# azrael417/mlperf-deepcam

Hardware: AMD Instinct MI355X
Metric: samples/sec (768x1152x16) train step (higher is better)
Workload: dtype bf16; 1 GPU; DeepLabV3+/Xception train step (fwd + weighted CE + bwd + LAMB), 768x1152x16, local_batch=8, bf16 activations / fp32 master weights, random-init seed 333; local_batch=8, global_batch=8, parallelism=dp1, optimizer=LAMB, hip_graph=False, launch_list_replay=False

## Files before the change

mlperf-deepcam_amd/csrc/igemm224.hip:

```cpp
#include <type_traits>

#include "igemm.h"

namespace dc {

namespace {

constexpr int NWS = 3, NPS = 3;
constexpr int NPB = 7;
constexpr int PW224_AUXP = 0;

typedef __attribute__((address_space(1))) const void* gas_ptr;
typedef __attribute__((address_space(3))) void* lds_ptr;
typedef __attribute__((ext_vector_type(2))) uint32_t u32x2;
typedef __attribute__((ext_vector_type(4))) uint32_t u32x4;

__device__ inline uint32_t swap_rows16(uint32_t v) { return (uint32_t)__builtin_amdgcn_ds_swizzle((int)v, 0x401F); }
__device__ inline float row_sum16(float v) {
  v += __int_as_float(__builtin_amdgcn_update_dpp(0, __float_as_int(v), 0xB1, 0xF, 0xF, true));
  v += __int_as_float(__builtin_amdgcn_update_dpp(0, __float_as_int(v), 0x4E, 0xF, 0xF, true));
  v += __int_as_float(__builtin_amdgcn_update_dpp(0, __float_as_int(v), 0x141, 0xF, 0xF, true));
  v += __int_as_float(__builtin_amdgcn_update_dpp(0, __float_as_int(v), 0x140, 0xF, 0xF, true));
  return v;
}

__device__ inline void mfma_v(f32x4& c, const bf16x8& av, const bf16x8& bv) {
  asm volatile("v_mfma_f32_16x16x32_bf16 %0, %1, %2, %0" : "+v"(c) : "v"(av), "v"(bv));
}
template <int OFF>
__device__ inline void lds_read16(bf16x8& dst, uint32_t addr) {
  static_assert(OFF >= 0 && OFF < 65536, "ds_read offset field");
  asm volatile("ds_read_b128 %0, %1 offset:%2" : "=v"(dst) : "v"(addr), "n"(OFF) : "memory");
}
template <int OFF>
__device__ inline void lds_read_tr(u32x4& dst, uint32_t addr) {
  static_assert(OFF >= 0 && OFF + 512 < 65536, "ds_read offset field");
  u32x2 lo, hi;
  asm volatile("ds_read_b64_tr_b16 %0, %1 offset:%2" : "=v"(lo) : "v"(addr), "n"(OFF) : "memory");
  asm volatile("ds_read_b64_tr_b16 %0, %1 offset:%2" : "=v"(hi) : "v"(addr), "n"(OFF + 512) : "memory");
  dst[0] = lo[0]; dst[1] = lo[1]; dst[2] = hi[0]; dst[3] = hi[1];
}
template <int N>
__device__ inline void lgkm_wait() {
  asm volatile("s_waitcnt lgkmcnt(%0)" ::"n"(N) : "memory");
}
template <int N>
__device__ inline void vm_lgkm0_wait() {
  asm volatile("s_waitcnt vmcnt(%0) lgkmcnt(0)" ::"n"(N) : "memory");
}

template <int I, int N, typename F>
__device__ inline void static_for(F&& f) {
  if constexpr (I < N) {
    f(std::integral_constant<int, I>{});
    static_for<I + 1, N>(f);
  }
}

template <int TN_>
struct Cfg {
  static constexpr int TN = TN_;
  static constexpr int GP = 2;
  static constexpr int GC = 8 / GP;
  static constexpr int NCB = TN / 16 / GC;
  static constexpr int TM = GP * NPB * 16;
  static constexpr int WSTG = 32 * TN * 2;
  static constexpr int NWI = WSTG / 1024;
  static constexpr int WSLOTS = (NWI + 7) / 8;
  static constexpr int WDEF = (NWI % 8) ? 1 : 0;
  static constexpr int PSTG = TM * 128;
  static constexpr int NPI = PSTG / 1024;
  static constexpr int PSLOTS = (NPI + 7) / 8;
  static constexpr int HP = PSLOTS / 2;
  static constexpr int POFF = NWS * WSTG;
  static constexpr int RING = NWS * WSTG + NPS * PSTG;
  static_assert(PSLOTS % 2 == 0 && NCB % 3 == 0 && RING <= 160 * 1024, "plan");
  static_assert(NPI - 8 * (PSLOTS - 1) == 4 && (WDEF == 0 || NWI - 8 * (WSLOTS - 1) == 4), "waves 0..3 own every last slot");
};

template <int TNT>
__global__ __launch_bounds__(512) void pw224_kernel(const IgemmParams p) {
  typedef Cfg<TNT> K;
  constexpr int NCB = K::NCB, GC = K::GC, HP = K::HP, TN = K::TN, WSTG = K::WSTG, GP = K::GP;
  extern __shared__ __attribute__((aligned(16))) char smem[];
  const GatherGeom& g = p.g;
  const int tid = threadIdx.x, lane = tid & 63;
  const int wave = __builtin_amdgcn_readfirstlane(tid >> 6);
  const int grp = wave / GC;
  const int wc = wave % GC;
  const bool late = wave >= 4;

  const int ntn = (g.Cout + TN - 1) / TN;
  const int nwg = gridDim.x;
  const int q8 = nwg >> 3, r8 = nwg & 7, xcd = blockIdx.x & 7, xslot = blockIdx.x >> 3;
  const int tile = (xcd < r8 ? xcd * (q8 + 1) : r8 * (q8 + 1) + (xcd - r8) * q8) + xslot;
  const int tm = tile / ntn;
  const int n0 = (tile % ntn) * TN, m0 = tm * K::TM;
  const int nsteps = (g.Cin + 31) / 32;

  const int krow = 8 * (wave & 3) + (lane >> 3);
  const int wkey = ((krow >> 1) & 1) | (((krow >> 3) & 1) << 1);
  unsigned srcw[K::WSLOTS], srcp[K::PSLOTS];
#pragma unroll
  for (int i = 0; i < K::WSLOTS; ++i) {
    const int ncol = ((wave >> 2) + 2 * i) * 64 + ((((lane & 7) >> 1) ^ wkey) << 4) + (lane & 1) * 8;
    srcw[i] = (unsigned)(((size_t)krow * p.ldw_kn + n0 + ncol) * 2);
// ... 77 lines not shown
        static_for<0, ND>([&](auto kc) {
          constexpr int k = decltype(kc)::value;
          if constexpr (EB[k] == i) { if (!late) dma_k(kc); }
          if constexpr (LB[k] == i) { if (late) dma_k(kc); }
        });
      }
      if constexpr (i == NCB - 1) {
        if (dma) {
          if (has_last) vm_lgkm0_wait<K::WSLOTS + HP>(); else vm_lgkm0_wait<K::WSLOTS + HP - K::WDEF - H>();
        } else {
          vm_lgkm0_wait<0>();
        }
        __builtin_amdgcn_s_barrier();
        lds_read_tr<0>(fa[0], wnxt + a_base[0] - lds0);
        lds_read_tr<0>(fa[1], wnxt + a_base[1] - lds0);
      }
      static_for<0, NPB>([&](auto jc) {
        constexpr int j = decltype(jc)::value;
        if constexpr (i == 0) lgkm_wait<NPB - 1 - j + 2>();
        else if constexpr (j == 0 && i < NCB - 2) lgkm_wait<4>();
        else if constexpr (j == 0 && i == NCB - 2) lgkm_wait<2>();
        mfma_v(acc[i][j], __builtin_bit_cast(bf16x8, fa[i % 3]), fb[j]);
        if constexpr (i == NCB - 1) lds_read16<j * 2048>(fb[j], bnxt);
      });
    });
  };

  constexpr int LATE_PRIO = 1;
  if (late) __builtin_amdgcn_s_setprio(LATE_PRIO);
#pragma unroll
  for (int q = 0; q < 2; ++q) {
#pragma unroll
    for (int i = 0; i < K::PSLOTS; ++i)
      if (i < K::PSLOTS - 1 || has_last) issue_p(i, q, K::POFF + q * K::PSTG);
#pragma unroll
    for (int i = 0; i < K::WSLOTS; ++i)
      if (i < K::WSLOTS - K::WDEF || has_last) issue_w(i, q, q * WSTG);
  }
  if (has_last) asm volatile("s_waitcnt vmcnt(%0)" ::"n"(K::WSLOTS + K::PSLOTS) : "memory");
  else asm volatile("s_waitcnt vmcnt(%0)" ::"n"(K::WSLOTS - K::WDEF + K::PSLOTS - 1) : "memory");
  __builtin_amdgcn_s_barrier();
  lds_read_tr<0>(fa[0], a_base[0]);
  lds_read_tr<0>(fa[1], a_base[1]);
  static_for<0, NPB>([&](auto jc) { lds_read16<decltype(jc)::value * 2048>(fb[decltype(jc)::value], lds0 + b_off); });
  {
    int s = 0;
    uint32_t w0 = 0, w1 = WSTG, w2 = 2 * WSTG;
    uint32_t p0 = 0, p1 = K::PSTG, p2 = 2 * K::PSTG;
    typedef std::integral_constant<int, 0> H0;
    typedef std::integral_constant<int, 1> H1;
    while (true) {
      step(H0{}, lds0 + w0, lds0 + w1, lds0 + ((b_off + p0) ^ 64), s, s + 2 < nsteps, w2, K::POFF + p2);
      if (++s == nsteps) break;
      step(H1{}, lds0 + w1, lds0 + w2, lds0 + b_off + p1, s, s + 2 < nsteps, w0, K::POFF + p2);
      if (++s == nsteps) break;
      { const uint32_t t = w0; w0 = w2; w2 = w1; w1 = t; }
      { const uint32_t t = p0; p0 = p1; p1 = p2; p2 = t; }
    }
  }
  asm volatile("s_waitcnt vmcnt(0) lgkmcnt(0)" ::: "memory");

  __builtin_amdgcn_s_barrier();

  const bool odd = fg & 1;
  bf16* __restrict__ yg = reinterpret_cast<bf16*>(p.y);
  const bool do_stats = p.slab != nullptr;
  float* red = reinterpret_cast<float*>(smem);
#pragma unroll
  for (int pr = 0; pr < NCB / 2; ++pr) {
    const int i0 = 2 * pr;
    const int cpair = TN == 384 ? ((wc >> 1) + 2 * pr) * 64 + (wc & 1) * 32 : 48 * wc;
    const int chl = cpair + (odd ? 16 : 0) + (fg >> 1) * 8;
    const int ch0 = n0 + chl;
    const bool chok = ch0 < g.Cout;
    float ba[4] = {0.f, 0.f, 0.f, 0.f}, bb[4] = {0.f, 0.f, 0.f, 0.f};
    if (p.bias != nullptr) {
#pragma unroll
      for (int r = 0; r < 4; ++r) {
        const int ca = n0 + cpair + fg * 4 + r, cb = ca + 16;
        if (ca < g.Cout) ba[r] = p.bias[ca];
        if (cb < g.Cout) bb[r] = p.bias[cb];
      }
    }
    float st[2][8];
#pragma unroll
    for (int e = 0; e < 8; ++e) st[0][e] = st[1][e] = 0.f;
#pragma unroll
    for (int j = 0; j < NPB; ++j) {
      const int m = m0 + grp * (NPB * 16) + j * 16 + fr;
      const uint32_t a0 = pack2_bf16(acc[i0][j][0] + ba[0], acc[i0][j][1] + ba[1]);
      const uint32_t a1 = pack2_bf16(acc[i0][j][2] + ba[2], acc[i0][j][3] + ba[3]);
      const uint32_t b0 = pack2_bf16(acc[i0 + 1][j][0] + bb[0], acc[i0 + 1][j][1] + bb[1]);
      const uint32_t b1 = pack2_bf16(acc[i0 + 1][j][2] + bb[2], acc[i0 + 1][j][3] + bb[3]);
      const uint32_t r0 = swap_rows16(odd ? a0 : b0), r1 = swap_rows16(odd ? a1 : b1);
      vec16 v;
      v.w[0] = odd ? r0 : a0;
      v.w[1] = odd ? r1 : a1;
      v.w[2] = odd ? b0 : r0;
      v.w[3] = odd ? b1 : r1;
      if (m < p.M && chok) {
        bf16* dst = yg + (size_t)m * p.ldy + ch0;
        float f[8];
        unpack(v, f, bf16());
        if (p.accumulate) {
          float o[8];
          unpack(ldg16(dst), o, bf16());
#pragma unroll
          for (int e = 0; e < 8; ++e) f[e] += o[e];
          pack(v, f, bf16());
          unpack(v, f, bf16());
        }
        stg16(dst, v);
        if (do_stats) {
#pragma unroll
          for (int e = 0; e < 8; ++e) {
            st[0][e] += f[e];
            st[1][e] = fmaf(f[e], f[e], st[1][e]);
          }
        }
      }
    }
    if (do_stats) {
      float mine = 0.f;
#pragma unroll
      for (int w = 0; w < 2; ++w)
#pragma unroll
        for (int e = 0; e < 8; ++e) {
          const float t = row_sum16(st[w][e]);
          if (fr == w * 8 + e) mine = t;
        }
      red[(grp * 2 + (fr >> 3)) * TN + chl + (fr & 7)] = mine;
    }
  }
  if constexpr (NCB & 1) {
    constexpr int i2 = NCB - 1;
    const int chl = 48 * wc + 32 + (fg >> 1) * 8;
    const int ch0 = n0 + chl;
    const bool chok = ch0 < g.Cout;
    float ba[4] = {0.f, 0.f, 0.f, 0.f};
    if (p.bias != nullptr) {
#pragma unroll
      for (int r = 0; r < 4; ++r) {
        const int ca = n0 + 48 * wc + 32 + fg * 4 + r;
        if (ca < g.Cout) ba[r] = p.bias[ca];
      }
    }
    float st[2][8];
#pragma unroll
    for (int e = 0; e < 8; ++e) st[0][e] = st[1][e] = 0.f;
#pragma unroll
    for (int jj = 0; jj < (NPB + 1) / 2; ++jj) {
      const int j0 = 2 * jj, j1 = 2 * jj + 1 < NPB ? 2 * jj + 1 : 2 * jj;
      const bool has1 = 2 * jj + 1 < NPB;
      const uint32_t a0 = pack2_bf16(acc[i2][j0][0] + ba[0], acc[i2][j0][1] + ba[1]);
      const uint32_t a1 = pack2_bf16(acc[i2][j0][2] + ba[2], acc[i2][j0][3] + ba[3]);
      const uint32_t b0 = pack2_bf16(acc[i2][j1][0] + ba[0], acc[i2][j1][1] + ba[1]);
      const uint32_t b1 = pack2_bf16(acc[i2][j1][2] + ba[2], acc[i2][j1][3] + ba[3]);
      const uint32_t r0 = swap_rows16(odd ? a0 : b0), r1 = swap_rows16(odd ? a1 : b1);
      vec16 v;
      v.w[0] = odd ? r0 : a0;
      v.w[1] = odd ? r1 : a1;
      v.w[2] = odd ? b0 : r0;
      v.w[3] = odd ? b1 : r1;
      const int m = m0 + grp * (NPB * 16) + (odd ? j1 : j0) * 16 + fr;
      if (m < p.M && chok && (!odd || has1)) {
        bf16* dst = yg + (size_t)m * p.ldy + ch0;
        float f[8];
        unpack(v, f, bf16());
        if (p.accumulate) {
          float o[8];
          unpack(ldg16(dst), o, bf16());
#pragma unroll
          for (int e = 0; e < 8; ++e) f[e] += o[e];
          pack(v, f, bf16());
          unpack(v, f, bf16());
        }
        stg16(dst, v);
        if (do_stats) {
#pragma unroll
          for (int e = 0; e < 8; ++e) {
            st[0][e] += f[e];
            st[1][e] = fmaf(f[e], f[e], st[1][e]);
          }
        }
      }
    }
    if (do_stats) {
      float mine = 0.f;
#pragma unroll
      for (int w = 0; w < 2; ++w)
#pragma unroll
        for (int e = 0; e < 8; ++e) {
          const float both = st[w][e] + __uint_as_float(swap_rows16(__float_as_uint(st[w][e])));
          const float t = row_sum16(both);
          if (fr == w * 8 + e) mine = t;
        }
      if (!odd) red[(grp * 2 + (fr >> 3)) * TN + chl + (fr & 7)] = mine;
    }
  }
  if (do_stats) {
    __syncthreads();
    const int rows = p.mtiles, ntm = (p.M + K::TM - 1) / K::TM;
    for (int i = tid; i < 2 * TN; i += 512) {
      const int c = i % TN, which = i / TN;
      if (n0 + c < g.Cout) {
        float v = red[which * TN + c];
#pragma unroll
        for (int gq = 1; gq < GP; ++gq) v += red[(gq * 2 + which) * TN + c];
        if (rows < 0) {
          unsafeAtomicAdd(reinterpret_cast<double*>(p.slab) + (size_t)which * g.Cout + n0 + c, (double)v);
          continue;
        }
        float* col = p.slab + (size_t)which * rows * g.Cout + n0 + c;
        col[(size_t)tm * g.Cout] = v;
        for (int r = tm + ntm; r < rows; r += ntm) col[(size_t)r * g.Cout] = 0.f;
      }
    }
  }
}

}

bool pw224_eligible(const IgemmParams& p) {
  const GatherGeom& g = p.g;
  return p.w_kn != nullptr && g.ntaps == 1 && g.os == 1 && g.is == 1 && g.taps[0].dy == 0 && g.taps[0].dx == 0 && p.m_beg == 0 && p.ngroup <= 1 &&
         g.Cin >= 128 && g.Cin % 8 == 0 && g.Cout % 8 == 0 && (((uintptr_t)p.w_kn) & 15) == 0 &&
         ((size_t)p.M + 224) * p.ldx * 2 < (1ull << 31) && ((size_t)g.Cin + 64) * p.ldw_kn * 2 < (1ull << 31);
}

int launch_pw224(const IgemmParams& p, int tn, hipStream_t st) {
  auto k384 = &pw224_kernel<384>;
  auto k192 = &pw224_kernel<192>;
  DC_ONCE({
    (void)hipFuncSetAttribute(reinterpret_cast<const void*>(k384), hipFuncAttributeMaxDynamicSharedMemorySize, Cfg<384>::RING);
    (void)hipFuncSetAttribute(reinterpret_cast<const void*>(k192), hipFuncAttributeMaxDynamicSharedMemorySize, Cfg<192>::RING);
  });
  if (tn == 192) hipLaunchKernelGGL(k192, dim3((unsigned)pw224_tiles(p, 192)), dim3(512), Cfg<192>::RING, st, p);
  else hipLaunchKernelGGL(k384, dim3((unsigned)pw224_tiles(p, 384)), dim3(512), Cfg<384>::RING, st, p);
  DC_CHECK_LAUNCH();
  return 0;
}

}
```

mlperf-deepcam_amd/engine.py:

```python
from __future__ import annotations

import ctypes as C
import math
from typing import Callable, Dict, List, Optional

import torch

from . import lib as L
from . import spec as S

BN_EPS = 1e-5
BN_MOMENTUM = 0.1
S_STEM_W = "xception_features.conv1.weight"
ACT_ALIGN = 64
BN_FIN_MAX_M = 16384
WGRAD_GROUP = 12


class Act:

    def __init__(self, eng: "Engine", name: str, N: int, H: int, W: int, Cc: int, parent: "Act" = None, off: int = 0,
                 dtype=None):
        self.eng, self.name, self.N, self.H, self.W, self.C = eng, name, N, H, W, Cc
        self.parent, self.off = parent, off
# ... 48 lines not shown
            init = init or a.grad_init
            a = a.parent
        self.grad_init = True
        self.grad_takes += 1
        return 1 if init else 0


class LazyAct:

    def __init__(self, y: Act, scale: torch.Tensor, shift: torch.Tensor, mean: torch.Tensor, invstd: torch.Tensor, relu: bool,
                 fin: Optional[dict], name: str):
        self.y, self.scale, self.shift, self.mean, self.invstd, self.relu, self.name = y, scale, shift, mean, invstd, relu, name
        self.N, self.H, self.W, self.C = y.N, y.H, y.W, y.C
        self._grad: Optional[Act] = None
        self.grad_init = False
        self.fin = fin
        self.fused_bwd: Optional[tuple] = None
        self.apply_by: Optional[Callable] = None

    @property
    def M(self) -> int:
        return self.y.M

    @property
    def grad(self) -> Act:
        if self._grad is None:
            self._grad = Act(self.y.eng, "d" + self.name, self.N, self.H, self.W, self.C, dtype=self.y.buf.dtype)
        return self._grad

    def take_grad_mode(self) -> int:
        mode = 1 if self.grad_init else 0
        self.grad_init = True
        return mode


class Engine:
    def __init__(self, batch: int, height: int, width: int, dtype=torch.bfloat16, device=None, n_input: int = 16,
                 n_classes: int = 3, seed: Optional[int] = 333, share_from: "Engine" = None, layout: "S.Layout" = None,
                 builder: Callable[["Engine"], None] = None, frozen_bn: bool = False, fuse_bn_into_head: bool = True):
        if not torch.cuda.is_available():
            raise L.DeepcamHipError("mlperf_deepcam_amd.Engine needs a HIP device: there is no CPU path")
        L.load()
        assert n_classes == 3, "the fused loss / head kernels are built for the 3 DeepCAM classes"
        assert height % 16 == 0 and width % 16 == 0, "input extents must be multiples of the output stride (16)"
        self.B, self.H, self.W = batch, height, width
        self.dtype, self.dt = dtype, L.dtype_code(dtype)
        self.device = device or torch.device("cuda", torch.cuda.current_device())
        self.n_input, self.n_classes = n_input, n_classes
        self.layout = layout if layout is not None else S.Layout(n_input, n_classes)
        self._builder = builder
        lay = self.layout
        self.act_bytes = 0
        self.saved: Dict[str, torch.Tensor] = {}
        self.saved_channels: Dict[str, int] = {}

        if share_from is not None:
            assert share_from.layout.n_params == lay.n_params and share_from.device == self.device
            self.params, self.grads, self.buffers, self.nbt = share_from.params, share_from.grads, share_from.buffers, share_from.nbt
            self.version = share_from.version
            self.grads_live = share_from.grads_live
        else:
            host = torch.empty(lay.n_params, dtype=torch.float32)
            if layout is None:
                S.init_arena(lay, host, seed)
            else:
                host.zero_()
            self.params = host.to(self.device)
            self.grads = torch.zeros(lay.n_params, dtype=torch.float32, device=self.device)
            hb = torch.zeros(lay.n_buffers, dtype=torch.float32)
            for name, (off, c) in lay.buffers.items():
                if name.endswith("running_var"):
                    hb[off:off + c] = 1.0
            self.buffers = hb.to(self.device)
            self.nbt = torch.zeros(len(lay.nbt), dtype=torch.int64, device=self.device)
            self.version = [0]
            self.grads_live = [False]
        self.packed_version = -1
        self._keep: List[torch.Tensor] = []
        self.frozen_bn = frozen_bn
        self.fuse_bn = not frozen_bn
        self.fuse_bn_into_head = fuse_bn_into_head and self.fuse_bn and dtype == torch.bfloat16
        self._sum_arena = None
        self._sum_used = 0
        self._wg_recs: List[dict] = []
        self._fold_seq: List[tuple] = []
        self._final_fold = None
        self._deferred_names: List[str] = []
        self._ready_now: List[str] = []
        self._stem_out: Optional[Act] = None
        self._layout_op: Optional[Callable[[], None]] = None
        self._layout_forked = False

        self.fwd_train: List[Callable[[], None]] = []
        self.fwd_eval: List[Callable[[], None]] = []
        self.bwd: List[Callable[[], None]] = []
        self.pack_ops: List[Callable[[], None]] = []
        self._pack_entries: List[L.PackEntry] = []
        self.grad_ready: List[List[str]] = []
        self.ws_bytes = 0
        self._ws_users: List[Callable[[], int]] = []
        self.x_in: Optional[torch.Tensor] = None
        self.x0: Optional[Act] = None
        self.x_static = torch.empty((batch, n_input, height, width), dtype=torch.float32, device=self.device)
        self.logits = torch.empty((batch, n_classes, height, width), dtype=torch.float32, device=self.device)
        self.dlogits = torch.empty_like(self.logits)
        self._build()
        self.workspace = torch.empty(max(self.ws_bytes, 256), dtype=torch.uint8, device=self.device)
        arr = (L.PackEntry * len(self._pack_entries))(*self._pack_entries)
        raw = torch.frombuffer(bytearray(bytes(arr)), dtype=torch.uint8).clone()
        self._pack_table = raw.to(self.device)
        npk = len(self._pack_entries)
        self.pack_ops.append(lambda: L.call("dc_pack_all", self.dt, L.dptr(self._pack_table), npk, self._st()))
        self.side = torch.cuda.Stream(device=self.device)
        self.workspace2 = torch.empty(max(self.ws_bytes, 256), dtype=torch.uint8, device=self.device)
        self.use_side_stream = True
        self.on_grad_ready: Optional[Callable[[List[str]], None]] = None
        self.region_marks: Optional[list] = None
        self.loss_args: Optional[dict] = None

    def pptr(self, name: str) -> C.c_void_p:
        return C.c_void_p(self.params.data_ptr() + self.layout.params[name].offset * 4)

    def gptr(self, name: str) -> C.c_void_p:
        return C.c_void_p(self.grads.data_ptr() + self.layout.params[name].offset * 4)

    def bptr(self, name: str) -> C.c_void_p:
        return C.c_void_p(self.buffers.data_ptr() + self.layout.buffers[name][0] * 4)

    def param_view(self, name: str) -> torch.Tensor:
        p = self.layout.params[name]
        return self.params[p.offset:p.offset + math.prod(p.shape)].view(p.shape)

    def grad_view(self, name: str) -> torch.Tensor:
        p = self.layout.params[name]
        return self.grads[p.offset:p.offset + math.prod(p.shape)].view(p.shape)

    def buffer_view(self, name: str) -> torch.Tensor:
        if name in self.layout.nbt:
            return self.nbt[self.layout.nbt[name]]
        off, c = self.layout.buffers[name]
        return self.buffers[off:off + c]

    def _need_ws(self, nbytes: int) -> None:
        self.ws_bytes = max(self.ws_bytes, int(nbytes))

    def _wsptr(self) -> C.c_void_p:
        return C.c_void_p(self.workspace.data_ptr())

    def _on_side(self, fn: Callable[[C.c_void_p], None]) -> None:
        if not self.use_side_stream:
            fn(self._wsptr())
            return
        L.call("dc_stream_fence", L.stream_ptr(), C.c_void_p(self.side.cuda_stream))
        with torch.cuda.stream(self.side):
            fn(C.c_void_p(self.workspace2.data_ptr()))

    @staticmethod
    def _st():
        return L.stream_ptr()

    def _f32(self, n: int) -> torch.Tensor:
        return torch.empty(n, dtype=torch.float32, device=self.device)

    SUM_ARENA_FLOATS = 1 << 21

    def _sum_row(self, channels: int) -> torch.Tensor:
        if self._sum_arena is None:
            self._sum_arena = torch.zeros(self.SUM_ARENA_FLOATS, dtype=torch.float32, device=self.device)
        n = (4 * channels + 15) // 16 * 16
        if self._sum_used + n > self.SUM_ARENA_FLOATS:
            raise L.DeepcamHipError("the arena of BatchNorm sum rows is full (Engine.SUM_ARENA_FLOATS)")
        row = self._sum_arena[self._sum_used:self._sum_used + n]
        self._sum_used += n
        return row

    def _conv(self, x: Act, wname: str, cout: int, k: int = 1, stride: int = 1, pad: int = 0, dil: int = 1,
              transposed: bool = False, out: Act = None, stats: bool = True, bias: str = None, name: str = None,
              need_dx: bool = True, f32: bool = False, fwd_group: list = None, sole_consumer: bool = False, bn_fuse: bool = False,
              sum_row: bool = True):
        lib = L.load()
        dt, tdtype = (L.DC_F32, torch.float32) if f32 else (self.dt, self.dtype)
        d = L.ConvDesc(dt, 3 if transposed else k, stride, pad, dil, 1 if transposed else 0, x.C, cout)
        ho, wo = C.c_int(), C.c_int()
        L.call("dc_conv_out_hw", C.byref(d), x.H, x.W, C.byref(ho), C.byref(wo))
        y = out or Act(self, name or wname, x.N, ho.value, wo.value, cout, dtype=tdtype)
        assert (y.H, y.W, y.C) == (ho.value, wo.value, cout) and y.buf.dtype == tdtype and x.buf.dtype == tdtype
        nwf, nwb = C.c_size_t(), C.c_size_t()
        L.call("dc_conv_packed_elems", C.byref(d), C.byref(nwf), C.byref(nwb))
        wf = torch.empty(nwf.value, dtype=tdtype, device=self.device)
        wb = torch.empty(nwb.value, dtype=tdtype, device=self.device) if need_dx else None
        both = k == 1 and stride == 1 and not transposed and not f32 and need_dx and dt == L.DC_BF16
        rows = (lib.dc_conv_stat_rows_kn if both else lib.dc_conv_stat_rows)(C.byref(d), x.N, x.H, x.W) if stats else 0
        slab = self._f32(2 * rows * cout) if stats else None
        if (stats and both and sum_row and self.fuse_bn and fwd_group is None and bias is None and out is None
                and lib.dc_conv_sum_row_kn(C.byref(d), x.N, x.H, x.W) == 1):
            rows, slab = -1, self._sum_row(cout)
        if (bn_fuse and self.fuse_bn and k == 1 and stride == 1 and not transposed and bias is None and not f32 and need_dx
                and out is None and x.parent is None):
            frows = lib.dc_pw_bn_bwd_rows(dt, x.C, cout, x.M)
            if frows > 0:
                y.pw_fuse = {"rows": frows, "taken": False}
        N, H, W = x.N, x.H, x.W
        pw, gw = self.pptr(wname), self.gptr(wname)
        pb = self.pptr(bias) if bias else None
        if f32 and self.dt != L.DC_F32:
            self.pack_ops.append(lambda: L.call("dc_conv_pack_weights", C.byref(d), pw, L.dptr(wf), L.dptr(wb), self._st()))
        else:
            self._pack_entries.append(L.PackEntry(pw.value, wf.data_ptr(), wb.data_ptr() if wb is not None else None, x.C, cout,
                                                  d.k * d.k, 1 if transposed else 0))
            self._keep += [wf] + ([wb] if wb is not None else [])

        assert both == (k == 1 and stride == 1 and not transposed and not f32 and wb is not None and dt == L.DC_BF16)

        def fwd(train: bool):
            if both:
                L.call("dc_conv_fwd_kn", C.byref(d), N, H, W, x.ptr, x.ld, L.dptr(wf), L.dptr(wb), pb, y.ptr, y.ld,
                       L.dptr(slab) if train else None, rows, 0, self._st())
            else:
                L.call("dc_conv_fwd", C.byref(d), N, H, W, x.ptr, x.ld, L.dptr(wf), pb, y.ptr, y.ld,
                       L.dptr(slab) if train else None, 0, self._st())

        if fwd_group is not None:
            assert k == 3 and stride == 1 and pad == dil and not transposed and bias is None and not f32
            fwd_group.append((dil, wf, y, slab, d, x))
        else:
            self.fwd_train.append(lambda: fwd(True))
            self.fwd_eval.append(lambda: fwd(False))
            y.conv_fwd = {"wf": wf, "slab": slab, "rows": rows, "plain": k == 1 and stride == 1 and not transposed and bias is None and not f32 and out is None}

        def make_bwd():
            pwf = y.pw_fuse
            if pwf is not None and pwf["taken"]:
                mode = x.take_grad_mode()
                assert mode == 0, f"{wname}: the fused backward pass writes the input gradient first"
                dx, do = x.grad, pwf["do"]
                frows = pwf["rows"]
                fslab = self._f32(frows * cout * x.C)
                ready = [wname] + pwf["names"]
                self._fold_seq.append(("dw", L.FoldEntry(fslab.data_ptr(), gw.value, L.DC_FOLD_CONV, frows, 1, cout, x.C), wname, ready))

                def bwd_fused():
                    L.call("dc_pw_bn_bwd", dt, y.M, x.C, cout, y.M, do.ptr, do.ld, y.ptr, y.ld, pwf["relu"], pwf["gam"], L.dptr(pwf["mean"]),
                           L.dptr(pwf["invstd"]), pwf["dgam"], pwf["dbet"], L.dptr(pwf["scale"]), L.dptr(pwf["shift"]), x.ptr, x.ld, L.dptr(wb),
                           dx.ptr, dx.ld, L.dptr(fslab), frows, self._st())
                return bwd_fused, ready
            dy = y.grad
            mode = x.take_grad_mode() if need_dx else 0
            dx = x.grad if need_dx else None
            ready = [wname] + ([bias] if bias else [])
            if bias:
                self._need_ws(lib.dc_colsum_workspace(y.M, cout))

            bsrc = x.bn_src if (sole_consumer and need_dx) else None
            srows = lib.dc_conv_dgrad_bnstats_rows(C.byref(d), N, H, W) if (bsrc is not None and mode == 0 and x.parent is None) else 0
# ... 50 lines not shown
                    for op in ops:
                        op()
                    return
                L.call("dc_stream_fence", L.stream_ptr(), C.c_void_p(self.side.cuda_stream))
                with torch.cuda.stream(self.side):
                    for op in ops:
                        op()
            lst.append(forked)

    def _dilated_group_fwd(self, members: list) -> None:
        cnt = len(members)
        d0, x = members[0][4], members[0][5]
        y0 = members[0][2]
        assert all(m[5] is x and m[2].ld == y0.ld and (m[2].H, m[2].W, m[2].C) == (y0.H, y0.W, y0.C) for m in members)
        dils = (C.c_int * cnt)(*[m[0] for m in members])
        wfs = (C.c_void_p * cnt)(*[m[1].data_ptr() for m in members])
        slabs = (C.c_void_p * cnt)(*[m[3].data_ptr() for m in members])
        N, H, W = x.N, x.H, x.W
        wsb = L.load().dc_conv_fwd_dilated_group_workspace(C.byref(d0), N, H, W, cnt, dils) if self.dt == L.DC_BF16 else 0
        kws = torch.empty(wsb, dtype=torch.uint8, device=self.device) if wsb > 0 else None
        if kws is not None:
            self._keep.append(kws)

        def fwd(train: bool):
            ys = (C.c_void_p * cnt)(*[m[2].ptr.value for m in members])
            if kws is not None:
                L.call("dc_conv_fwd_dilated_group_ws", C.byref(d0), N, H, W, cnt, dils, x.ptr, x.ld, wfs, ys, y0.ld, slabs if train else None,
                       L.dptr(kws), wsb, self._st())
                return
            L.call("dc_conv_fwd_dilated_group", C.byref(d0), N, H, W, cnt, dils, x.ptr, x.ld, wfs, ys, y0.ld, slabs if train else None,
                   self._st())

        self.fwd_train.append(lambda: fwd(True))
        self.fwd_eval.append(lambda: fwd(False))

    def _dw(self, x, wname: str, stride: int, dil: int, name: str) -> Act:
        lib = L.load()
        lazy = isinstance(x, LazyAct)
        src = x.y if lazy else x
        ps = L.dptr(x.scale) if lazy else None
        psh = L.dptr(x.shift) if lazy else None
        prelu = (1 if x.relu else 0) if lazy else 0
        if lazy:
            self._keep += [x.scale, x.shift]
        Ho, Wo = (x.H - 1) // stride + 1, (x.W - 1) // stride + 1
        y = Act(self, name, x.N, Ho, Wo, x.C)
        N, H, W, Cc = x.N, x.H, x.W, x.C
        pm, gw = self.pptr(wname), self.gptr(wname)
        wpk = self._f32(9 * Cc)
        self._keep.append(wpk)
        pw = L.dptr(wpk)
        self._pack_entries.append(L.PackEntry(pm.value, wpk.data_ptr(), None, Cc, Cc, 9, 2))
        self._need_ws(lib.dc_dwconv_wgrad_workspace(Cc, N, H, W, stride))

        def fwd():
            L.call("dc_dwconv_fwd", self.dt, Cc, stride, dil, N, H, W, src.ptr, src.ld, pw, y.ptr, y.ld, ps, psh, prelu, self._st())

        fwd_train = fwd
        fin = x.fin if lazy else None
        if fin is not None and not fin["taken"] and lib.dc_dwconv_fwd_fin_ok(self.dt, Cc, stride, dil, N, H, W):
            fin["taken"] = True

            def fwd_train():
                L.call("dc_dwconv_fwd_fin", self.dt, Cc, stride, dil, N, H, W, src.ptr, src.ld, pw, y.ptr, y.ld, prelu, *fin["args"], self._st())
        else:
            fin = None
        self.fwd_train.append(fwd_train)
        self.fwd_eval.append(fwd)
        y.dw_fwd = {"fin": fin is not None, "src": src, "ps": ps, "psh": psh, "prelu": prelu, "taps": pw, "stride": stride, "dil": dil}

        def make_bwd():
            dy = y.grad
            mode = x.take_grad_mode()
            dx = x.grad
            srows = lib.dc_dwconv_dgrad_bnstats_rows(self.dt, Cc, stride, dil, N, H, W) if (lazy and mode == 0) else 0
            wrows = 0
            if srows == 0:
                wrows = lib.dc_dwconv_dgrad_wgrad_rows(self.dt, Cc, stride, dil, N, H, W)
            sum_ok = lib.dc_dwconv_dgrad_sum_row_ok(self.dt, Cc, stride, dil, N, H, W) == 1
            stats_sum = False
            if srows > 0:
                wrows = lib.dc_dwconv_dgrad_wgrad_rows(self.dt, Cc, stride, dil, N, H, W)
                stats_sum = sum_ok and wrows > 0
                sslab = self._sum_row(Cc) if stats_sum else self._f32(2 * srows * Cc)
                x.fused_bwd = (sslab, -1 if stats_sum else srows)
                mean_p, invstd_p = L.dptr(x.mean), L.dptr(x.invstd)
            res = x.bn_res if (not lazy and wrows > 0 and srows == 0) else None
            if res is not None and x.fused_bwd is None and x.parent is None and \
                    lib.dc_dwconv_dgrad_wgrad_bnres_rows(self.dt, Cc, stride, dil, N, H, W) == wrows:
                rslab2 = self._sum_row(Cc) if sum_ok else self._f32(2 * wrows * Cc)
                x.fused_bwd = (rslab2, -1 if sum_ok else wrows, x.grad_takes)
            else:
                res = None
            bsrc = x.bn_src if (not lazy and res is None and wrows > 0 and srows == 0 and stride == 1) else None
            if bsrc is not None and x.fused_bwd is None and x.parent is None:
                bslab2 = self._f32(2 * wrows * Cc)
                x.fused_bwd = (bslab2, wrows, x.grad_takes)
            else:
                bsrc = None
            fuse_state = {"res": res, "bsrc": bsrc}
            if res is not None or bsrc is not None:
                x.fused_bwd_cancel = lambda: fuse_state.update(res=None, bsrc=None)
            ready = [wname]
            if wrows > 0:
                wslab = self._f32(wrows * 9 * Cc)
                self._fold_seq.append(("dw", L.FoldEntry(wslab.data_ptr(), gw.value, L.DC_FOLD_DW, wrows, 9, Cc, 1), wname, ready))

            def dw_wgrad(ws):
                L.call("dc_dwconv_wgrad", self.dt, Cc, stride, dil, N, H, W, src.ptr, src.ld, dy.ptr, dy.ld, ws, gw, ps, psh, prelu, self._st())

            def bwd():
                res = fuse_state["res"]
                if res is not None:
                    L.call("dc_dwconv_dgrad_wgrad_bnres_sum" if sum_ok else "dc_dwconv_dgrad_wgrad_bnres", self.dt, Cc, stride, dil, N, H, W, dy.ptr, dy.ld, pw, dx.ptr if mode else None, dx.ld,
                           dx.ptr, dx.ld, src.ptr, src.ld, L.dptr(wslab), res["y"].ptr, res["y"].ld, L.dptr(res["mean"]), L.dptr(res["invstd"]),
                           res["relu"], L.dptr(rslab2), self._st())
                    return
                bs = fuse_state["bsrc"]
                if bs is not None:
                    L.call("dc_dwconv_dgrad_bnstats_wgrad_add", self.dt, Cc, stride, dil, N, H, W, dy.ptr, dy.ld, pw, dx.ptr if mode else None, dx.ld,
                           dx.ptr, dx.ld, bs["y"].ptr, bs["y"].ld, L.dptr(bs["mean"]), L.dptr(bs["invstd"]), L.dptr(bs["scale"]), L.dptr(bs["shift"]),
                           bs["relu"], L.dptr(bslab2), L.dptr(wslab), self._st())
                    return
                if wrows > 0 and srows == 0:
                    L.call("dc_dwconv_dgrad_wgrad", self.dt, Cc, stride, dil, N, H, W, dy.ptr, dy.ld, pw, dx.ptr if mode else None, dx.ld,
                           dx.ptr, dx.ld, src.ptr, src.ld, ps, psh, prelu, L.dptr(wslab), self._st())
                    return
                if wrows > 0:
                    L.call("dc_dwconv_dgrad_bnstats_wgrad_sum" if stats_sum else "dc_dwconv_dgrad_bnstats_wgrad", self.dt, Cc, stride, dil, N, H, W, dy.ptr, dy.ld, pw, dx.ptr, dx.ld, src.ptr, src.ld,
                           mean_p, invstd_p, ps, psh, prelu, L.dptr(sslab), L.dptr(wslab), self._st())
                    return
                self._on_side(dw_wgrad)
                if srows > 0:
                    L.call("dc_dwconv_dgrad_bnstats", self.dt, Cc, stride, dil, N, H, W, dy.ptr, dy.ld, pw, dx.ptr, dx.ld, src.ptr, src.ld,
                           mean_p, invstd_p, ps, psh, prelu, L.dptr(sslab), self._st())
                else:
                    L.call("dc_dwconv_dgrad", self.dt, Cc, stride, dil, N, H, W, dy.ptr, dy.ld, pw, dx.ptr if mode else None, dx.ld,
                           dx.ptr, dx.ld, self._st())
            return bwd, ready

        self.bwd.append(make_bwd)
        return y

    def _bn(self, y: Act, slab: torch.Tensor, rows: int, bname: str, relu: bool, residual: Act = None, out: Act = None,
            name: str = None, lazy: bool = False):
        lib = L.load()
        Cc, M = y.C, y.M
        assert not (lazy and (residual is not None or out is not None))
        bdt = L.dtype_code(y.buf.dtype)
        if lazy:
            o = None
        else:
            o = out or Act(self, name or bname, y.N, y.H, y.W, Cc, dtype=y.buf.dtype)
            assert o.buf.dtype == y.buf.dtype
        scale, shift, mean, invstd = (self._f32(Cc) for _ in range(4))
        for suffix, t in ((".scale", scale), (".shift", shift), (".save_mean", mean), (".save_invstd", invstd)):
            self.saved[bname + suffix] = t
        gam, bet = self.pptr(bname + ".weight"), self.pptr(bname + ".bias")
        rm, rv = self.bptr(bname + ".running_mean"), self.bptr(bname + ".running_var")
        nbt = C.c_void_p(self.nbt.data_ptr() + 8 * self.layout.nbt[bname + ".num_batches_tracked"])
        relu_i = 1 if relu else 0
        rptr = (lambda: residual.ptr) if residual is not None else (lambda: None)
        rld = residual.ld if residual is not None else 0

        fin = None
        if self.fuse_bn and (rows == -1 or (rows <= lib.dc_bn_bwd_apply_fin_max_rows() and M <= BN_FIN_MAX_M)):
            fin = {"taken": False, "args": (M, L.dptr(slab), rows, gam, bet, rm, rv, nbt, BN_MOMENTUM, BN_EPS, L.dptr(scale), L.dptr(shift),
                                            L.dptr(mean), L.dptr(invstd))}

        def fwd_train():
            if fin is not None and (fin["taken"] or not lazy):
                if not lazy:
                    L.call("dc_bn_apply_fin", bdt, M, Cc, M, y.ptr, y.ld, *fin["args"][1:], rptr(), rld, relu_i, o.ptr, o.ld, self._st())
                return
            L.call("dc_bn_finalize", Cc, M, L.dptr(slab), rows, gam, bet, rm, rv, nbt, BN_MOMENTUM, BN_EPS, L.dptr(scale),
                   L.dptr(shift), L.dptr(mean), L.dptr(invstd), self._st())
            if not lazy:
                L.call("dc_bn_apply", bdt, M, Cc, y.ptr, y.ld, L.dptr(scale), L.dptr(shift), rptr(), rld, relu_i, o.ptr, o.ld, self._st())

        def fwd_eval():
            L.call("dc_bn_eval_coeffs", Cc, gam, bet, rm, rv, BN_EPS, L.dptr(scale), L.dptr(shift), self._st())
            if not lazy:
                L.call("dc_bn_apply", bdt, M, Cc, y.ptr, y.ld, L.dptr(scale), L.dptr(shift), rptr(), rld, relu_i, o.ptr, o.ld, self._st())

        lz = LazyAct(y, scale, shift, mean, invstd, relu, fin, (name or bname) + ".lazy") if lazy else None
        if self.fuse_bn and not lazy and out is None:
            if residual is None:
                o.bn_src = {"y": y, "scale": scale, "shift": shift, "mean": mean, "invstd": invstd, "relu": relu_i}
            else:
                o.bn_res = {"y": y, "mean": mean, "invstd": invstd, "relu": relu_i}

        self.fwd_train.append(fwd_train)
        self.fwd_eval.append(fwd_eval)
        brows = lib.dc_bn_stat_rows(M)
        bsum = self.fuse_bn and Cc >= 256
        if bsum:
            brows, bslab = -1, self._sum_row(Cc)
        else:
            bslab = self._f32(2 * brows * Cc)

        def make_bwd():
            apply_by = lz.apply_by if lazy else None
            do = None if apply_by is not None else (lz.grad if lazy else o.grad)
            assert y.take_grad_mode() == 0, "a conv output feeds exactly one BatchNorm"
            g_out = None
            if residual is not None:
                assert residual.take_grad_mode() == 0, f"{bname}: residual gradient must be first written here"
                g_out = residual.grad
            dgam, dbet = self.gptr(bname + ".weight"), self.gptr(bname + ".bias")
            from_y = lazy or (relu and residual is None)
            mrelu = (2 if relu else 0) if from_y else relu_i
            optr = (lambda: None) if from_y else (lambda: o.ptr)
            old_ = 0 if from_y else o.ld
            if self.frozen_bn:
                assert not lazy and y.pw_fuse is None and o.fused_bwd is None
                dyf = y.grad

                def bwd_frozen():
                    L.call("dc_bn_bwd_frozen", bdt, M, Cc, do.ptr, do.ld, y.ptr, y.ld, optr(), old_, mrelu, gam, rm, rv, BN_EPS, dyf.ptr, dyf.ld,
                           g_out.ptr if g_out is not None else None, g_out.ld if g_out is not None else 0, L.dptr(bslab), L.dptr(scale),
                           L.dptr(shift), self._st())
                    L.call("dc_bn_bwd_finalize", Cc, L.dptr(bslab), brows, dgam, dbet, self._st())
                return bwd_frozen, [bname + ".weight", bname + ".bias"]
            pwf = y.pw_fuse if (apply_by is None and residual is None and mrelu in (0, 2)) else None
            if pwf is not None:
                pwf.update(taken=True, do=do, gam=gam, mean=mean, invstd=invstd, dgam=dgam, dbet=dbet, scale=scale, shift=shift, relu=mrelu,
                           names=[bname + ".weight", bname + ".bias"])
            dy = None if pwf is not None else y.grad

            fused = (lz if lazy else o).fused_bwd
            if fused is not None and len(fused) > 2 and o.grad_takes != fused[2]:
                if o.fused_bwd_cancel is None:
                    raise L.DeepcamHipError(f"{bname}: a consumer took this BatchNorm's backward sums but is not the last writer of the gradient")
                o.fused_bwd_cancel()
                fused = None
            rslab, rrows = (fused[0], fused[1]) if fused is not None else (bslab, brows)
            fin_in_apply = (apply_by is None and pwf is None
                            and (rrows == -1 or (rrows <= lib.dc_bn_bwd_apply_fin_max_rows() and M <= BN_FIN_MAX_M)))

            def bwd():
                if fused is None:
                    L.call("dc_bn_bwd_reduce_sum" if bsum else "dc_bn_bwd_reduce", bdt, M, Cc, do.ptr, do.ld, y.ptr, y.ld, optr(), old_, mrelu, L.dptr(mean),
                           L.dptr(invstd), L.dptr(bslab), L.dptr(scale), L.dptr(shift), self._st())
                if fin_in_apply:
                    L.call("dc_bn_bwd_apply_fin", bdt, M, Cc, M, do.ptr, do.ld, y.ptr, y.ld, optr(), old_, mrelu, gam, L.dptr(mean),
                           L.dptr(invstd), L.dptr(rslab), rrows, dgam, dbet, dy.ptr, dy.ld, g_out.ptr if g_out is not None else None,
                           g_out.ld if g_out is not None else 0, L.dptr(scale), L.dptr(shift), self._st())
                    return
                L.call("dc_bn_bwd_finalize", Cc, L.dptr(rslab), rrows, dgam, dbet, self._st())
                if pwf is not None:
                    return
                if apply_by is not None:
                    apply_by(gam, dgam, dbet, dy)
                    return
                L.call("dc_bn_bwd_apply", bdt, M, Cc, M, do.ptr, do.ld, y.ptr, y.ld, optr(), old_, mrelu, gam, L.dptr(mean),
                       L.dptr(invstd), dgam, dbet, dy.ptr, dy.ld, g_out.ptr if g_out is not None else None,
                       g_out.ld if g_out is not None else 0, L.dptr(scale), L.dptr(shift), self._st())
            return bwd, ([] if pwf is not None else [bname + ".weight", bname + ".bias"])

        self.bwd.append(make_bwd)
        return lz if lazy else o

    def _sep(self, x, s: S.SepSpec, residual: Act = None, relu_override: Optional[bool] = None, lazy: bool = False):
        d = self._dw(x, s.prefix + ".conv1.weight", s.stride, s.dil, s.prefix + ".dw")
        sep_cand = L.load().dc_sepconv_fwd_rows(self.dt, d.C, s.cout, s.stride, s.dil, d.N, d.H, d.W) > 0
        y, slab, rows = self._conv(d, s.prefix + ".pointwise.weight", s.cout, stats=bool(s.bn), name=s.prefix + ".pw",
                                   bn_fuse=bool(s.bn) and residual is None, sum_row=not sep_cand)
        dwf, cvf = d.dw_fwd, y.conv_fwd
        if (not dwf["fin"] and cvf["plain"] and d.parent is None and
                L.load().dc_sepconv_fwd_rows(self.dt, d.C, s.cout, dwf["stride"], dwf["dil"], d.N, d.H, d.W) > 0 and
                (slab is None or L.load().dc_sepconv_fwd_rows(self.dt, d.C, s.cout, 1, 1, d.N, d.H, d.W) <= rows)):
            src, wf_t = dwf["src"], cvf["wf"]
            if slab is not None:
                rows = L.load().dc_sepconv_fwd_rows(self.dt, d.C, s.cout, 1, 1, d.N, d.H, d.W)

            def sepconv_fwd(train: bool):
                L.call("dc_sepconv_fwd", self.dt, d.C, s.cout, d.N, d.H, d.W, src.ptr, src.ld, dwf["ps"], dwf["psh"], dwf["prelu"], dwf["taps"],
                       d.ptr, d.ld, L.dptr(wf_t), y.ptr, y.ld, L.dptr(slab) if (train and slab is not None) else None, rows if slab is not None else 0,
                       self._st())
            del self.fwd_train[-2:]
# ... 290 lines not shown
                continue
            rec = item[1]
            if rec["role"] == "defer":
                continue
            ents = [it[1] for it in pending] + rec["own_entries"]
            rec["fold"] = ((L.FoldEntry * len(ents))(*ents), len(ents))
            for _, _, name, ready in pending:
                ready.remove(name)
                rec["ready"].append(name)
            pending = []
        if pending:
            ents = [it[1] for it in pending]
            for _, _, name, ready in pending:
                ready.remove(name)
                self._deferred_names.append(name)
            self._final_fold = ((L.FoldEntry * len(ents))(*ents), len(ents), [it[2] for it in pending])

    def pack_weights(self) -> None:
        for op in self.pack_ops:
            op()
        self.packed_version = self.version[0]

    def mark_weights_changed(self) -> None:
        self.version[0] += 1

    def forward(self, x_nchw: torch.Tensor, train: bool = True) -> torch.Tensor:
        train = train and not self.frozen_bn
        if (self.x0 is not None and x_nchw.dim() == 4 and tuple(x_nchw.shape) == (self.B, self.H, self.W, self.n_input)
                and x_nchw.dtype == self.dtype and x_nchw.is_contiguous() and x_nchw.device == self.device):
            self.x0.buf = x_nchw
            self.x_in = None
            return self._run_forward(train)
        if self.x0 is not None:
            self.x0.buf = self._x0_own
        if tuple(x_nchw.shape) != (self.B, self.n_input, self.H, self.W):
            raise L.DeepcamHipError(f"engine built for input {(self.B, self.n_input, self.H, self.W)}, got {tuple(x_nchw.shape)}")
        if train and self.B * (self.H // 16) * (self.W // 16) < 1:
            raise ValueError("empty batch")
        if train and self.B < 2:
            raise ValueError("Expected more than 1 value per channel when training, got input size torch.Size([1, 256, 1, 1])")
        if x_nchw.dtype != torch.float32 or not x_nchw.is_contiguous() or x_nchw.device != self.device:
            x_nchw = x_nchw.to(device=self.device, dtype=torch.float32).contiguous()
        self.x_in = x_nchw
        return self._run_forward(train)

    def input_grad(self, out: Optional[torch.Tensor] = None) -> torch.Tensor:
        c1 = self._stem_out
        if c1 is None:
            raise L.DeepcamHipError("input_grad: this engine has no network stem (a custom layout)")
        shape = (self.B, self.n_input, self.H, self.W)
        if out is None:
            out = torch.empty(shape, dtype=torch.float32, device=self.device)
        if tuple(out.shape) != shape or out.dtype != torch.float32 or not out.is_contiguous() or out.device != self.device:
            raise L.DeepcamHipError(f"input_grad: out must be a contiguous fp32 tensor {shape} on {self.device}")
        dy = c1.grad
        L.call("dc_stem_dgrad", self.dt, self.B, self.n_input, self.H, self.W, dy.ptr, dy.ld, self.pptr(S_STEM_W), L.dptr(out), self._st())
        return out

    def _run_forward(self, train: bool) -> torch.Tensor:
        if train and self.B < 2:
            raise ValueError("Expected more than 1 value per channel when training, got input size torch.Size([1, 256, 1, 1])")
        if self.packed_version != self.version[0]:
            if self.use_side_stream and self.x_in is not None and self._layout_op is not None:
                L.call("dc_stream_fence", L.stream_ptr(), C.c_void_p(self.side.cuda_stream))
                with torch.cuda.stream(self.side):
                    self._layout_op()
                self._layout_forked = True
            self.pack_weights()
        marks = self.region_marks if train else None
        if marks is not None:
            marks.append(("fwd_begin", torch.cuda.current_stream().record_event(torch.cuda.Event(enable_timing=True))))
        if train and self._sum_used:
            L.call("dc_memset_async", L.dptr(self._sum_arena), 0, 4 * self._sum_used, self._st())
        for i, op in enumerate(self.fwd_train if train else self.fwd_eval):
            if marks is not None and i == self._enc_fwd_end:
                marks.append(("fwd_enc_end", torch.cuda.current_stream().record_event(torch.cuda.Event(enable_timing=True))))
            op()
        return self.logits

    def backward(self) -> None:
        cb = self.on_grad_ready
        marks = self.region_marks
        enc_begin = len(self.bwd) - self._enc_bwd_makers
        for i, (op, ready) in enumerate(zip(self.bwd, self.grad_ready)):
            if marks is not None and i == enc_begin:
                marks.append(("bwd_enc_begin", torch.cuda.current_stream().record_event(torch.cuda.Event(enable_timing=True))))
            op()
            if self._ready_now:
                ready, self._ready_now = ready + self._ready_now, []
            if cb is not None and ready:
                cb(ready)
        if self._final_fold is not None:
            ents, nent, names = self._final_fold
            self._on_side(lambda ws: L.call("dc_fold_slabs", ents, nent, self._st()))
            self._ready_now += names
        if self._ready_now:
            ready, self._ready_now = self._ready_now, []
            if cb is not None:
                cb(ready)
        if self.use_side_stream:
            L.call("dc_stream_fence", C.c_void_p(self.side.cuda_stream), L.stream_ptr())
        if marks is not None:
            marks.append(("bwd_end", torch.cuda.current_stream().record_event(torch.cuda.Event(enable_timing=True))))
```

Baseline: 263.3 samples/s.

## Use reduce-scatter DPP for BN stats epilogue and split backward sum-row arena

Replaces the per-channel 16-way DPP row sums, which were repeated for every channel and then selected per lane, with a butterfly reduce-scatter. Each step halves the live values per lane, so the number of DPP ops and adds drops. Statistics are now taken directly from the packed bf16 words, before the swizzle, as packed f32x2 FMA, and the redundant unpack on the non-accumulate path is removed. Separately, backward BN sum rows are allocated from the top of the arena and zeroed with their own memset at the start of backward, instead of sharing the forward-zeroed region. This may fix or avoid stale accumulation, and it adds one memset per step.

```diff
diff --git a/mlperf-deepcam_amd/csrc/igemm224.hip b/mlperf-deepcam_amd/csrc/igemm224.hip
--- a/mlperf-deepcam_amd/csrc/igemm224.hip
+++ b/mlperf-deepcam_amd/csrc/igemm224.hip
@@ -16,12 +16,29 @@
 typedef __attribute__((ext_vector_type(4))) uint32_t u32x4;
 
 __device__ inline uint32_t swap_rows16(uint32_t v) { return (uint32_t)__builtin_amdgcn_ds_swizzle((int)v, 0x401F); }
-__device__ inline float row_sum16(float v) {
-  v += __int_as_float(__builtin_amdgcn_update_dpp(0, __float_as_int(v), 0xB1, 0xF, 0xF, true));
-  v += __int_as_float(__builtin_amdgcn_update_dpp(0, __float_as_int(v), 0x4E, 0xF, 0xF, true));
-  v += __int_as_float(__builtin_amdgcn_update_dpp(0, __float_as_int(v), 0x141, 0xF, 0xF, true));
-  v += __int_as_float(__builtin_amdgcn_update_dpp(0, __float_as_int(v), 0x140, 0xF, 0xF, true));
-  return v;
+
+__device__ inline int rs_index(int fr) {
+  const int b2 = (fr >> 2) & 1, b3 = fr >> 3;
+  return ((fr ^ b2) & 1) | ((((fr >> 1) ^ b2) & 1) << 1) | ((b2 ^ b3) << 2) | (b3 << 3);
+}
+template <int CTRL, int LIVE>
+__device__ inline void rs_step(float* x, bool hi) {
+#pragma unroll
+  for (int k = 0; k < LIVE / 2; ++k) {
+    const float keep = hi ? x[2 * k + 1] : x[2 * k], give = hi ? x[2 * k] : x[2 * k + 1];
+    x[k] = keep + __int_as_float(__builtin_amdgcn_update_dpp(0, __float_as_int(give), CTRL, 0xF, 0xF, true));
+  }
+}
+template <int N>
+__device__ inline float row_reduce_scatter16(float (&x)[N], int fr) {
+  static_assert(N == 16 || N == 8, "values per lane");
+  const int v = rs_index(fr);
+  rs_step<0xB1, N>(x, v & 1);
+  rs_step<0x4E, N / 2>(x, (v >> 1) & 1);
+  rs_step<0x141, N / 4>(x, (v >> 2) & 1);
+  if constexpr (N == 16) rs_step<0x140, 2>(x, v >> 3);
+  else x[0] += __int_as_float(__builtin_amdgcn_update_dpp(0, __float_as_int(x[0]), 0x140, 0xF, 0xF, true));
+  return x[0];
 }
 
 __device__ inline void mfma_v(f32x4& c, const bf16x8& av, const bf16x8& bv) {
@@ -265,9 +282,9 @@
         if (cb < g.Cout) bb[r] = p.bias[cb];
       }
     }
-    float st[2][8];
-#pragma unroll
-    for (int e = 0; e < 8; ++e) st[0][e] = st[1][e] = 0.f;
+    f32x2 st[2][4];
+#pragma unroll
+    for (int k = 0; k < 4; ++k) st[0][k] = st[1][k] = f32x2{0.f, 0.f};
 #pragma unroll
     for (int j = 0; j < NPB; ++j) {
       const int m = m0 + grp * (NPB * 16) + j * 16 + fr;
@@ -281,38 +298,37 @@
       v.w[1] = odd ? r1 : a1;
       v.w[2] = odd ? b0 : r0;
       v.w[3] = odd ? b1 : r1;
+      if (do_stats && m < p.M) {
+        const uint32_t own[4] = {a0, a1, b0, b1};
+#pragma unroll
+        for (int k = 0; k < 4; ++k) {
+          const f32x2 f = {__uint_as_float(own[k] << 16), __uint_as_float(own[k] & 0xffff0000u)};
+          st[0][k] += f;
+          st[1][k] = __builtin_elementwise_fma(f, f, st[1][k]);
+        }
+      }
       if (m < p.M && chok) {
         bf16* dst = yg + (size_t)m * p.ldy + ch0;
-        float f[8];
-        unpack(v, f, bf16());
         if (p.accumulate) {
-          float o[8];
+          float f[8], o[8];
+          unpack(v, f, bf16());
           unpack(ldg16(dst), o, bf16());
 #pragma unroll
           for (int e = 0; e < 8; ++e) f[e] += o[e];
           pack(v, f, bf16());
-          unpack(v, f, bf16());
         }
         stg16(dst, v);
-        if (do_stats) {
-#pragma unroll
-          for (int e = 0; e < 8; ++e) {
-            st[0][e] += f[e];
-            st[1][e] = fmaf(f[e], f[e], st[1][e]);
-          }
-        }
       }
     }
     if (do_stats) {
-      float mine = 0.f;
+      float x[16];
 #pragma unroll
       for (int w = 0; w < 2; ++w)
 #pragma unroll
-        for (int e = 0; e < 8; ++e) {
-          const float t = row_sum16(st[w][e]);
-          if (fr == w * 8 + e) mine = t;
-        }
-      red[(grp * 2 + (fr >> 3)) * TN + chl + (fr & 7)] = mine;
+        for (int k = 0; k < 4; ++k) x[8 * w + 2 * k] = st[w][k][0], x[8 * w + 2 * k + 1] = st[w][k][1];
+      const int e = rs_index(fr);
+      const float mine = row_reduce_scatter16(x, fr);
+      red[(grp * 2 + (e >> 3)) * TN + cpair + ((e >> 2) & 1) * 16 + fg * 4 + (e & 3)] = mine;
     }
   }
   if constexpr (NCB & 1) {
@@ -331,6 +347,14 @@
     float st[2][8];
 #pragma unroll
     for (int e = 0; e < 8; ++e) st[0][e] = st[1][e] = 0.f;
+    auto add_stats = [&](float(&s8)[8], uint32_t w0, uint32_t w1) {
+      const float f[4] = {__uint_as_float(w0 << 16), __uint_as_float(w0 & 0xffff0000u), __uint_as_float(w1 << 16), __uint_as_float(w1 & 0xffff0000u)};
+#pragma unroll
+      for (int r = 0; r < 4; ++r) {
+        s8[r] += f[r];
+        s8[4 + r] = fmaf(f[r], f[r], s8[4 + r]);
+      }
+    };
 #pragma unroll
     for (int jj = 0; jj < (NPB + 1) / 2; ++jj) {
       const int j0 = 2 * jj, j1 = 2 * jj + 1 < NPB ? 2 * jj + 1 : 2 * jj;
@@ -339,6 +363,11 @@
       const uint32_t a1 = pack2_bf16(acc[i2][j0][2] + ba[2], acc[i2][j0][3] + ba[3]);
       const uint32_t b0 = pack2_bf16(acc[i2][j1][0] + ba[0], acc[i2][j1][1] + ba[1]);
       const uint32_t b1 = pack2_bf16(acc[i2][j1][2] + ba[2], acc[i2][j1][3] + ba[3]);
+      if (do_stats) {
+        const int mj = m0 + grp * (NPB * 16) + j0 * 16 + fr;
+        if (mj < p.M) add_stats(st[0], a0, a1);
+        if (has1 && mj + 16 < p.M) add_stats(st[1], b0, b1);
+      }
       const uint32_t r0 = swap_rows16(odd ? a0 : b0), r1 = swap_rows16(odd ? a1 : b1);
       vec16 v;
       v.w[0] = odd ? r0 : a0;
@@ -359,26 +388,15 @@
           unpack(v, f, bf16());
         }
         stg16(dst, v);
-        if (do_stats) {
-#pragma unroll
-          for (int e = 0; e < 8; ++e) {
-            st[0][e] += f[e];
-            st[1][e] = fmaf(f[e], f[e], st[1][e]);
-          }
-        }
       }
     }
     if (do_stats) {
-      float mine = 0.f;
-#pragma unroll
-      for (int w = 0; w < 2; ++w)
-#pragma unroll
-        for (int e = 0; e < 8; ++e) {
-          const float both = st[w][e] + __uint_as_float(swap_rows16(__float_as_uint(st[w][e])));
-          const float t = row_sum16(both);
-          if (fr == w * 8 + e) mine = t;
-        }
-      if (!odd) red[(grp * 2 + (fr >> 3)) * TN + chl + (fr & 7)] = mine;
+      float both[8];
+#pragma unroll
+      for (int e = 0; e < 8; ++e) both[e] = st[0][e] + st[1][e];
+      const int e = rs_index(fr) & 7;
+      const float mine = row_reduce_scatter16(both, fr);
+      if (fr < 8) red[(grp * 2 + (e >> 2)) * TN + 48 * wc + 32 + fg * 4 + (e & 3)] = mine;
     }
   }
   if (do_stats) {
diff --git a/mlperf-deepcam_amd/engine.py b/mlperf-deepcam_amd/engine.py
--- a/mlperf-deepcam_amd/engine.py
+++ b/mlperf-deepcam_amd/engine.py
@@ -154,6 +154,7 @@
         self.fuse_bn_into_head = fuse_bn_into_head and self.fuse_bn and dtype == torch.bfloat16
         self._sum_arena = None
         self._sum_used = 0
+        self._bwd_sum_used = 0
         self._wg_recs: List[dict] = []
         self._fold_seq: List[tuple] = []
         self._final_fold = None
@@ -236,12 +237,16 @@
 
     SUM_ARENA_FLOATS = 1 << 21
 
-    def _sum_row(self, channels: int) -> torch.Tensor:
+    def _sum_row(self, channels: int, backward: bool = False) -> torch.Tensor:
         if self._sum_arena is None:
             self._sum_arena = torch.zeros(self.SUM_ARENA_FLOATS, dtype=torch.float32, device=self.device)
         n = (4 * channels + 15) // 16 * 16
-        if self._sum_used + n > self.SUM_ARENA_FLOATS:
+        if self._sum_used + self._bwd_sum_used + n > self.SUM_ARENA_FLOATS:
             raise L.DeepcamHipError("the arena of BatchNorm sum rows is full (Engine.SUM_ARENA_FLOATS)")
+        if backward:
+            self._bwd_sum_used += n
+            end = self.SUM_ARENA_FLOATS - self._bwd_sum_used
+            return self._sum_arena[end:end + n]
         row = self._sum_arena[self._sum_used:self._sum_used + n]
         self._sum_used += n
         return row
@@ -458,13 +463,13 @@
             if srows > 0:
                 wrows = lib.dc_dwconv_dgrad_wgrad_rows(self.dt, Cc, stride, dil, N, H, W)
                 stats_sum = sum_ok and wrows > 0
-                sslab = self._sum_row(Cc) if stats_sum else self._f32(2 * srows * Cc)
+                sslab = self._sum_row(Cc, backward=True) if stats_sum else self._f32(2 * srows * Cc)
                 x.fused_bwd = (sslab, -1 if stats_sum else srows)
                 mean_p, invstd_p = L.dptr(x.mean), L.dptr(x.invstd)
             res = x.bn_res if (not lazy and wrows > 0 and srows == 0) else None
             if res is not None and x.fused_bwd is None and x.parent is None and \
                     lib.dc_dwconv_dgrad_wgrad_bnres_rows(self.dt, Cc, stride, dil, N, H, W) == wrows:
-                rslab2 = self._sum_row(Cc) if sum_ok else self._f32(2 * wrows * Cc)
+                rslab2 = self._sum_row(Cc, backward=True) if sum_ok else self._f32(2 * wrows * Cc)
                 x.fused_bwd = (rslab2, -1 if sum_ok else wrows, x.grad_takes)
             else:
                 res = None
@@ -571,7 +576,7 @@
         brows = lib.dc_bn_stat_rows(M)
         bsum = self.fuse_bn and Cc >= 256
         if bsum:
-            brows, bslab = -1, self._sum_row(Cc)
+            brows, bslab = -1, self._sum_row(Cc, backward=True)
         else:
             bslab = self._f32(2 * brows * Cc)
 
@@ -1028,6 +1033,9 @@
         cb = self.on_grad_ready
         marks = self.region_marks
         enc_begin = len(self.bwd) - self._enc_bwd_makers
+        if self._bwd_sum_used:
+            rows = self._sum_arena[self.SUM_ARENA_FLOATS - self._bwd_sum_used:]
+            L.call("dc_memset_async", L.dptr(rows), 0, 4 * self._bwd_sum_used, self._st())
         for i, (op, ready) in enumerate(zip(self.bwd, self.grad_ready)):
             if marks is not None and i == enc_begin:
                 marks.append(("bwd_enc_begin", torch.cuda.current_stream().record_event(torch.cuda.Event(enable_timing=True))))
```

New measurement: 263.7 samples/s (median of 6 runs). About the same (+0.1%).
